# giech/usrp_nfc

Measured on AMD Instinct MI355X. Metric: IQ Msamples/s -> decoded bits (2 Msps stream), higher is better.
Workload: dtype f32 envelope / f64 window sums / u8 symbols; 1 GPU; configs[1]: Miller-only decode, synthetic IQ @2 Msps; input_kind=fc32 IQ, 8 B/sample (envelope computed in the kernel), samples_per_gpu=100000000, parallelism=time-chunk x1, edges_per_gpu=6627699, symbols_reader=3971547, symbols_tag=0, packets=101186, boundary_redos=0, exchange=none, stepping=sync, in_flight=1

## Files before the change

### usrp_nfc_amd/csrc/decode.hip.h

```cpp
#pragma once
#include <hip/hip_runtime.h>
#include <stdint.h>

#include "../../include/nfc_amd.h"
#include "scan.hip.h"

namespace nfc {

struct DecTables {
    const uint4 *mil_map;
    const uint2 *man_map;
    const uint16_t *mil_step;
    const uint16_t *man_step;
    int32_t nd;
    int32_t reader, tag;
    const uint2 *qmil_map;
    const uint16_t *qmil_step;
    uint32_t q_rep[2];
    uint32_t canon[4];
    int32_t q_ok;
};
__device__ __forceinline__ uint32_t byte_of(const uint32_t *w, uint32_t i) { return (w[i >> 2] >> (8u * (i & 3u))) & 0xFFu; }

struct DecCarry {
    int32_t mil_state, man_state;
    int32_t pkt_started[2];
    uint32_t pending[2];
};

constexpr int DEC_ITEMS = 16;
#ifndef NFC_DEC_GROUPS
#define NFC_DEC_GROUPS 2
#endif
constexpr int DEC_GROUPS = NFC_DEC_GROUPS;
constexpr int DEC_PER_THREAD = DEC_ITEMS * DEC_GROUPS;
// ... 337 lines not shown
        v <<= (lo & 31u);
        if (v) atomicOr(dst + w0 + j, v);
    }
}

struct QMaps {
    uint32_t mil[2];
    uint32_t man[2];
};
struct ComposeQ {
    using T = QMaps;
    static __host__ __device__ __forceinline__ T identity() { return T{{0x03020100u, 0x07060504u}, {0x03020100u, 0x07060504u}}; }
    static __device__ __forceinline__ T op(const T &a, const T &b) {
        return T{{__builtin_amdgcn_perm(b.mil[1], b.mil[0], a.mil[0]), __builtin_amdgcn_perm(b.mil[1], b.mil[0], a.mil[1])},
                 {__builtin_amdgcn_perm(b.man[1], b.man[0], a.man[0]), __builtin_amdgcn_perm(b.man[1], b.man[0], a.man[1])}};
    }
    static __device__ __forceinline__ uint32_t step(const T &m, uint32_t st) {
        const uint32_t a = __builtin_amdgcn_perm(m.mil[1], m.mil[0], st & 7u) & 15u;
        const uint32_t b = __builtin_amdgcn_perm(m.man[1], m.man[0], (st >> 4) & 7u) & 15u;
        return a | (b << 4);
    }
};
struct DecSpec {
    QMaps map;
    uint32_t s_in;
    uint32_t needs;
    uint32_t pad[2];
};
static_assert(sizeof(DecSpec) == 32, "two 16-byte loads");
__device__ __forceinline__ bool map8_constant(const uint32_t (&m)[2]) { return m[0] == m[1] && m[0] == (m[0] & 0xFFu) * 0x01010101u; }
constexpr int DEC_RUNIN_MAX = 8;
static_assert(DEC_GROUPS >= 1 && DEC_GROUPS <= 2, "NFC_DEC_GROUPS: a thread's packed bits are accumulated in 64 bits (32 slots per group)");
static_assert(DEC_RUNIN_MAX * SCAN_BLOCK <= DEC_TILE, "the longest run-in fits inside the tile before");
template <bool LDS>
__global__ __launch_bounds__(SCAN_BLOCK) void k_dec_spec(const uint16_t *ecode, size_t n, const uint32_t *n_dev, DecTables T, uint32_t state0, int runin_per_thread,
                                                        uint8_t *outw, FrameAgg *frame_aggs, DecSpec *spec, ZeroJob Z, TileStage S) {
    zero_words(Z);
    if (n_dev) n = min(n, (size_t)*n_dev);
    if ((size_t)blockIdx.x * DEC_TILE >= n) return;
    TP_DECL();
    __shared__ uint2 s_milmap[LDS ? DEC_LDS_ROWS + 1 : 1];
    __shared__ uint2 s_manmap[LDS ? DEC_LDS_ROWS + 1 : 1];
    __shared__ __attribute__((aligned(16))) uint16_t s_mil[LDS ? DEC_LDS_ROWS * 8 : 8];
    __shared__ __attribute__((aligned(16))) uint16_t s_man[LDS ? DEC_LDS_ROWS * 8 : 8];
    __shared__ QMaps lds[SCAN_WAVES];
    __shared__ FramePk lds2[SCAN_WAVES];
    __shared__ uint32_t s_needs;
    __shared__ uint32_t s_bits[2][FW_WORDS];
    __shared__ uint32_t s_drop[2];
    for (int i = threadIdx.x; i < 2 * FW_WORDS; i += SCAN_BLOCK) (&s_bits[0][0])[i] = 0u;
    if (threadIdx.x < 2) s_drop[threadIdx.x] = 0xFFFFFFFFu;
    const uint32_t ident = 4u * (uint32_t)T.nd;
    if (LDS) {
        const int rows = 4 * T.nd;
        for (int i = threadIdx.x; i <= rows; i += SCAN_BLOCK) {
            if (T.reader) s_milmap[i] = T.qmil_map[i];
            if (T.tag) s_manmap[i] = T.man_map[i];
        }
        for (int i = threadIdx.x; i < rows; i += SCAN_BLOCK) {
            if (T.reader) ((uint4 *)s_mil)[i] = ((const uint4 *)T.qmil_step)[i];
            if (T.tag) ((uint4 *)s_man)[i] = ((const uint4 *)T.man_step)[i];
        }
    }
    if (threadIdx.x == 0) s_needs = 0u;
    const size_t tid = (size_t)blockIdx.x * SCAN_BLOCK + threadIdx.x;
    const size_t base = tid * DEC_PER_THREAD;
    uint32_t c[DEC_GROUPS][8];
#pragma unroll
    for (int g = 0; g < DEC_GROUPS; g++) load_codes(ecode, base + DEC_ITEMS * g, n, c[g]);
    uint32_t rc[DEC_RUNIN_MAX / 2];
    const bool have_runin = blockIdx.x > 0;
    {
        const size_t r0 = (size_t)blockIdx.x * DEC_TILE - (size_t)runin_per_thread * SCAN_BLOCK + (size_t)threadIdx.x * runin_per_thread;
#pragma unroll
        for (int k = 0; k < DEC_RUNIN_MAX / 2; k++) rc[k] = (have_runin && 2 * k < runin_per_thread) ? *(const uint32_t *)(ecode + r0 + 2 * k) : 0u;
    }
    __syncthreads();
    TP_MARK();
    auto mil_row = [&](uint32_t code) __attribute__((always_inline)) -> uint2 {
        const uint32_t idx = (code >> 14) == 2u ? (code & 0x3FFFu) : ident;
        return LDS ? s_milmap[idx] : T.qmil_map[idx];
    };
    auto man_row = [&](uint32_t code) __attribute__((always_inline)) -> uint2 {
        const uint32_t idx = (code >> 14) == 1u ? (code & 0x3FFFu) : ident;
        return LDS ? s_manmap[idx] : T.man_map[idx];
    };
    auto then = [](const uint2 &a, const uint2 &b) __attribute__((always_inline)) -> uint2 {
        return make_uint2(__builtin_amdgcn_perm(b.y, b.x, a.x), __builtin_amdgcn_perm(b.y, b.x, a.y));
    };
    auto routes_of = [](uint32_t pair) __attribute__((always_inline)) -> uint32_t {
        const uint32_t r0 = (pair >> 14) & 3u, r1 = pair >> 30;
        return ((r0 == 2u || r1 == 2u) ? 1u : 0u) | ((r0 == 1u || r1 == 1u) ? 2u : 0u);
    };
    auto compose4 = [&](uint2 &am, uint2 &an, uint32_t w0, uint32_t w1) __attribute__((always_inline)) {
        const uint32_t c0 = w0 & 0xFFFFu, c1 = w0 >> 16, c2 = w1 & 0xFFFFu, c3 = w1 >> 16;
        if (T.reader) am = then(am, then(then(mil_row(c0), mil_row(c1)), then(mil_row(c2), mil_row(c3))));
        if (T.tag) an = then(an, then(then(man_row(c0), man_row(c1)), then(man_row(c2), man_row(c3))));
    };
    const QMaps idm = ComposeQ::identity();
    QMaps runin = idm;
    if (have_runin) {
        uint2 am = make_uint2(idm.mil[0], idm.mil[1]), an = make_uint2(idm.man[0], idm.man[1]);
#pragma unroll
        for (int k = 0; k < DEC_RUNIN_MAX / 2; k += 2)
            if (2 * k < runin_per_thread) compose4(am, an, rc[k], rc[k + 1]);
        const QMaps ra{{am.x, am.y}, {an.x, an.y}};
        (void)block_exclusive<ComposeQ>(ra, lds, runin);
    }
    uint32_t seen = 0u;
    uint2 am = make_uint2(idm.mil[0], idm.mil[1]), an = make_uint2(idm.man[0], idm.man[1]);
#ifndef NFC_DEC_CHAIN
#define NFC_DEC_CHAIN 8
#endif
    constexpr int CHAIN = NFC_DEC_CHAIN;
    static_assert(CHAIN == 16 || CHAIN == 8 || CHAIN == 4, "NFC_DEC_CHAIN");
    constexpr int NCH = DEC_PER_THREAD / CHAIN;
    uint2 pm[NCH], pn[NCH];
#pragma unroll
    for (int g = 0; g < DEC_GROUPS; g++) {
#pragma unroll
        for (int k = 0; k < 8; k += 2) {
            if (k % (CHAIN / 2) == 0) {
                pm[(16 * g + 2 * k) / CHAIN] = am;
                pn[(16 * g + 2 * k) / CHAIN] = an;
            }
            compose4(am, an, c[g][k], c[g][k + 1]);
            seen |= routes_of(c[g][k]) | routes_of(c[g][k + 1]);
        }
    }
    if (!T.reader) seen &= ~1u;
    if (!T.tag) seen &= ~2u;
    const QMaps agg{{am.x, am.y}, {an.x, an.y}};
    TP_MARK();
    QMaps total;
    const QMaps excl = block_exclusive<ComposeQ>(agg, lds, total);
    const QMaps upto = ComposeQ::op(runin, excl);
    const uint32_t dep = ((seen & 1u) && !map8_constant(upto.mil) ? 1u : 0u) | ((seen & 2u) && !map8_constant(upto.man) ? 2u : 0u);
    if (blockIdx.x > 0 && dep) atomicOr(&s_needs, dep);
    uint32_t st[NCH];
#pragma unroll
    for (int j = 0; j < NCH; j++) st[j] = ComposeQ::step(ComposeQ::op(upto, QMaps{{pm[j].x, pm[j].y}, {pn[j].x, pn[j].y}}), state0);
    TP_MARK();
    const uint16_t *mil = LDS ? s_mil : T.qmil_step;
    const uint16_t *man = LDS ? s_man : T.man_step;
    uint32_t ow[DEC_GROUPS][4];
#pragma unroll
    for (int g = 0; g < DEC_GROUPS; g++) ow[g][0] = ow[g][1] = ow[g][2] = ow[g][3] = 0u;
#pragma unroll
    for (int e = 0; e < CHAIN; e++) {
#pragma unroll
        for (int j = 0; j < NCH; j++) {
            const int g = (j * CHAIN) / DEC_ITEMS, k = (j * CHAIN) % DEC_ITEMS + e;
            const uint32_t code = (c[g][k >> 1] >> (16 * (k & 1))) & 0xFFFFu;
            const uint32_t li = code & 0x3FFFu, route = code >> 14;
            uint32_t w = 0;
            if (route == 2u && T.reader) {
                const uint32_t en = mil[li * 8u + (st[j] & 7u)];
                w = en >> 8;
                st[j] = (st[j] & ~15u) | (en & 15u);
            } else if (route == 1u && T.tag) {
                const uint32_t en = man[li * 8u + ((st[j] >> 4) & 7u)];
                const uint32_t m = en >> 8;
                w = (m & 3u) ? ((m & 0xFCu) | 3u) : 0u;
                st[j] = (st[j] & 15u) | ((en & 15u) << 4);
            }
            ow[g][k >> 2] |= w << (8 * (k & 3));
        }
    }
    FramePk mine = FramePkOp::identity();
#pragma unroll
    for (int g = 0; g < DEC_GROUPS; g++) {
        const size_t gb = base + (size_t)DEC_ITEMS * g;
        if (gb < n) *(uint4 *)(outw + gb) = make_uint4(ow[g][0], ow[g][1], ow[g][2], ow[g][3]);
        mine = FramePkOp::op(mine, FramePkOp::pack(frame_agg_of(ow[g])));
    }
    TP_MARK();
    FramePk total_fa;
    const FramePk in_tile = block_exclusive<FramePkOp>(mine, lds2, total_fa);
    {
        FrameAgg before = FramePkOp::unpack(in_tile);
        uint64_t acc[2] = {0ull, 0ull};
        uint32_t cnt[2] = {0u, 0u};
        const uint32_t bo0[2] = {before.nb[0], before.nb[1]};
#pragma unroll
        for (int g = 0; g < DEC_GROUPS; g++) {
            if (ow[g][0] | ow[g][1] | ow[g][2] | ow[g][3]) {
                const SlotMasks m = slot_masks(ow[g]);
                const uint32_t low = symbol_low_bits(ow[g]);
#pragma unroll
                for (int t = 0; t < 2; t++) {
                    if (!m.V[t] || !S.bits[t]) continue;
                    const uint32_t started = pm_apply(before.fl[t], 1u);
                    const uint32_t bef = started_before(m, t, started);
                    const uint32_t appended = m.V[t] & ~m.ST[t] & (bef | ~m.SA[t]);
                    uint32_t cl = m.ST[t] & bef;
                    const uint32_t bo = bo0[t] + cnt[t];
                    const uint32_t nonid = m.ST[t] | m.SA[t];
                    if ((before.fl[t] & 3u) == PM_ID && nonid) {
                        const uint32_t first = nonid & (0u - nonid);
                        if (first & m.SA[t]) s_drop[t] = bo + (uint32_t)__popc(appended & (first - 1u));
                    }
                    acc[t] |= (uint64_t)compress32(low, appended) << cnt[t];
                    cnt[t] += (uint32_t)__popc(appended);
                    if (cl) {
                        const uint32_t co = before.nc[t], closes = cl;
                        while (cl) {
                            const uint32_t lowb = cl & (0u - cl);
                            const int k = (__ffs((int)cl) - 1) >> 1;
                            cl ^= lowb;
                            const uint32_t j = co + (uint32_t)__popc(closes & (lowb - 1u));
                            if (j < ST_CLOSES) {
                                const size_t e = base + (size_t)DEC_ITEMS * g + k;
                                S.close_bit[t][(size_t)blockIdx.x * ST_CLOSES + j] = bo + (uint32_t)__popc(appended & (lowb - 1u));
                                S.close_idx[t][(size_t)blockIdx.x * ST_CLOSES + j] = S.idx64 ? S.idx64[e] : S.g0 + (uint64_t)S.epos[e];
                            } else {
                                atomicOr(&s_needs, 4u);
                            }
                        }
                    }
                }
                if (g + 1 < DEC_GROUPS) before = FrameAggOp::op(before, frame_agg_of(ow[g]));
            }
        }
#pragma unroll
        for (int t = 0; t < 2; t++) {
            if (!cnt[t]) continue;
            const uint32_t w = bo0[t] >> 5, sh = bo0[t] & 31u;
            const uint64_t lo = acc[t] << sh;
            const uint32_t hi = sh ? (uint32_t)(acc[t] >> (64u - sh)) : 0u;
            if (w + 2 < (uint32_t)FW_WORDS) {
                if ((uint32_t)lo) atomicOr(&s_bits[t][w], (uint32_t)lo);
                if ((uint32_t)(lo >> 32)) atomicOr(&s_bits[t][w + 1], (uint32_t)(lo >> 32));
                if (hi) atomicOr(&s_bits[t][w + 2], hi);
            }
        }
    }
    __syncthreads();
    const FrameAgg tile_fa = FramePkOp::unpack(total_fa);
#pragma unroll
    for (int t = 0; t < 2; t++) {
        if (!S.bits[t]) continue;
        const uint32_t nw = min((uint32_t)FW_WORDS, (tile_fa.nb[t] + 31u) / 32u + 1u);
        for (uint32_t j = threadIdx.x; j < nw; j += SCAN_BLOCK) S.bits[t][(size_t)blockIdx.x * FW_WORDS + j] = s_bits[t][j];
    }
    if (threadIdx.x == 0) {
        frame_aggs[blockIdx.x] = tile_fa;
        S.own[blockIdx.x] = tile_fa;
        if (S.bits[0]) S.drop_bit[0][blockIdx.x] = s_drop[0];
        if (S.bits[1]) S.drop_bit[1][blockIdx.x] = s_drop[1];
        const uint32_t s_in = ComposeQ::step(runin, state0);
        ((uint4 *)(spec + blockIdx.x))[0] = make_uint4(total.mil[0], total.mil[1], total.man[0], total.man[1]);
        ((uint4 *)(spec + blockIdx.x))[1] = make_uint4(s_in, s_needs, 0u, 0u);
    }
    TP_DONE(1);
}

struct DecVerify {
    const DecSpec *spec;
    uint32_t state0;
    uint32_t q_rep[2];
    DecCarry *carry;
    uint32_t *verdict;
};
constexpr int DV_ITEMS = 4;
__device__ __forceinline__ void dec_verify(const DecVerify &V, size_t ntiles, QMaps *lds) {
    QMaps before = ComposeQ::identity();
    int bad = 0;
    for (size_t b0 = 0; b0 < ntiles; b0 += (size_t)SCAN_BLOCK * DV_ITEMS) {
        const size_t i0 = b0 + (size_t)threadIdx.x * DV_ITEMS;
        QMaps mp[DV_ITEMS];
        uint32_t s_in[DV_ITEMS], needs[DV_ITEMS];
#pragma unroll
        for (int k = 0; k < DV_ITEMS; k++) {
            if (i0 + k < ntiles) {
                const uint4 a = ((const uint4 *)(V.spec + i0 + k))[0], b = ((const uint4 *)(V.spec + i0 + k))[1];
                mp[k] = QMaps{{a.x, a.y}, {a.z, a.w}};
                s_in[k] = b.x;
                needs[k] = b.y;
            } else {
                mp[k] = ComposeQ::identity();
                s_in[k] = 0u;
                needs[k] = 0u;
            }
        }
        QMaps agg = mp[0];
// ... 396 lines not shown
```

### usrp_nfc_amd/csrc/host_context.h

```cpp
#pragma once


namespace {

std::string g_create_error;

__global__ __launch_bounds__(256) void k_certify_and_write(CertLaunch C, EdgeArgs E, size_t nwords, const EdgeAgg *partials, const EdgeAgg *supers,
                                                          uint32_t *epos, uint16_t *ecode, uint32_t cap, bool own_prefix, uint32_t *total_out,
                                                          Last2 *last2_total, EdgeCarry *carry_out) {
    const uint32_t tiles = gridDim.x - C.blocks;
    if (blockIdx.x == 0) {
        certify_block(C.A, C.cert, nullptr, C.ring_next, C.carry, C.sum, C.blocks - 1, C.blocks);
        return;
    }
    if (blockIdx.x > tiles) {
        certify_block(C.A, C.cert, nullptr, C.ring_next, C.carry, C.sum, blockIdx.x - tiles - 1, C.blocks);
        return;
    }
    write_edges_tile(E, nwords, partials, supers, epos, ecode, cap, own_prefix, total_out, last2_total, carry_out, tiles - blockIdx.x, tiles);
}

inline uint64_t &devbuf_allocs() {
    static thread_local uint64_t n = 0;
    return n;
// ... 40 lines not shown
    TOT_EDGES = 8,
    TOT_DECMAP = 16,
    TOT_SPEC = 40,
    TOT_PKT0 = 72,
    TOT_PKT1 = 80,
    TOT_LAST2 = 88,
    TOT_NSYM = 96,
    TOT_CERT = 104,
    TOT_FRAME = 128,
    TOT_BYTES = 160
};

static_assert(sizeof(CertSummary) <= TOT_FRAME - TOT_CERT, "the verdict summary fits its slot of the totals");
struct DevState {
    Carry carry;
    EdgeCarry ecarry;
    DecCarry dcarry;
    uint8_t totals[TOT_BYTES];
    uint32_t seq[4];
};

constexpr size_t AHEAD_LDS_MAX = 96 * 1024;
constexpr int NRING = 4;
constexpr int NSUB = 3;

struct nfc_ctx {
    nfc_params P;
    int L, mx, C, Lpad, wpb, twords;
    double factor;
    double hi_plus, lo_a, lo_b, hi_a, hi_b;
    int bands_ok, fast_ok, nfold, rows_per_step, C_min, wave_slots, lds_per_slot;
    uint32_t ring_carried = 0;
    bool dec_spec = true, dec_spec_now = false;
    int dec_runin = 2, spec_off_left = 0, spec_fail_streak = 0;
    bool bits_packed = false, sym_lazy = false, sym_own = false;
    FrameOut sym_P;
    uint32_t sym_n = 0, sym_tiles = 0;
    uint32_t decode_respeculated = 0;
    int lean = 1, lean_k = 0, lean_rounds = 0, lean_slots = 0;
    int n_cus = 1;
    double rowbal_f[5][3] = {{1, 1, 1}, {1, 1, 1}, {1.02, 1, 1}, {1.045, 1.004, 1}, {1.036, 1.015, 0.990}};
    bool rowbal_set = false;
    bool wg_rowbal = true, rowbal_now = false;
    int wg = 1, wg_ok = 0, wg_nr = 4, wg_slots = 0, wg_slots_ahead = 0, wg_now = 0, wg_rounds = 0;
    int fine_left = 0, fine_adapt = 1, fine_mult = 4;
    size_t wg_lds = 0, wg_lds_base = 0, wg_lds_bulk_max = 0;
    bool wg_bulk = true, wg_bulk_now = false;
    int wg_lone_max = 4, wg_lone_div = 64;
    int wg_rerun_lone = 1;
    int wg_ex_ok = 0, wg_ex_max = 0;
    size_t wg_ex_lds = 0;
    bool wg_ex_launch = false;
    bool wg_flags = false;
    float lean_gfac = 1.3f, lean_gmin = 9.765625e-4f;
    int gring = 0;
    int gring_ok = 0, gring_force = 0, wave_slots_g = 0;
    DevBuf d_gring;
    uint32_t own_prefix_max = OWN_PREFIX_MAX_TILES;
    int use_small = 1;
    double expect_ms = 0.3;
    bool spin_wait = true;
    uint64_t selmask;
    float eps;
    float i16_scale;
    size_t in_bytes_per_sample;
    hipStream_t st = nullptr;
// ... 398 lines not shown
```

### usrp_nfc_amd/csrc/host_stages.h

```cpp
#pragma once

namespace {

int run_edges(nfc_ctx *c, uint32_t n, uint32_t skip, uint64_t g0) {
    uint8_t *tot = dT(c);
    const size_t nwords = ((size_t)n + 63) / 64;
    EdgeArgs E;
    E.neg = c->d_neg.as<uint64_t>();
    E.pos = c->d_pos.as<uint64_t>();
    E.n = n;
    E.skip = skip;
    E.mx = c->mx;
    E.dur_in = c->h_ecarry.dur;
    E.last_bit_in = c->h_ecarry.last_bit;
    E.state_in = c->h_ecarry.state;
    E.nd = c->mx + 1;
    E.g0 = g0;
    E.mx_magic = c->mx > 1 ? (uint32_t)(0x100000000ull / (uint64_t)c->mx) : 0xFFFFFFFFu;
    E.per_mask = 0;
    for (int b = 0; b < 64; b += c->mx) E.per_mask |= 1ull << b;
    E.sw = (uint32_t)(EW_WORDS * EW_SUPER);
    E.tps = (uint32_t)EW_SUPER;
    const size_t tiles = edge_num_tiles(nwords);
    const size_t supers = edge_num_supers(nwords);
// ... 54 lines not shown
        P.pending[t] = c->d_pending[t][c->pend_cur].as<uint8_t>();
        P.pend[t] = pend;
    }
    return NFC_OK;
}

void launch_pkt_finish(nfc_ctx *c, const FrameOut &P, const bool (&enabled)[2], PktCnt *pk_total, FrameAgg *frame_total) {
    const int pn = 1 - c->pend_cur;
    PktFinish F;
    memset(&F, 0, sizeof F);
    F.packed = 1;
    for (int t = 0; t < 2; t++) {
        F.enabled[t] = enabled[t] ? 1 : 0;
        F.bits[t] = P.bits[t];
        F.pending_next[t] = c->d_pending[t][pn].as<uint8_t>();
        F.close_end[t] = P.close_end[t];
        F.started_in[t] = (int32_t)P.started_in[t];
        F.pending_cap[t] = (uint32_t)std::min<size_t>(c->d_pending[t][pn].cap, 0xFFFFFFFFu);
        F.cap_bits[t] = P.cap_bits[t];
        F.cap_close[t] = P.cap_close[t];
    }
    F.totals = pk_total;
    F.frame_total = frame_total;
    F.carry = dD(c);
    static_assert(sizeof(DevState) % 4 == 0, "whole words");
    F.mirror_src = (const uint32_t *)c->d_state.p;
    F.mirror_dst = (uint32_t *)c->hs_dev;
    F.mirror_words = (uint32_t)(sizeof(DevState) / 4);
    F.stamp_word = (uint32_t)(offsetof(DevState, seq) / 4 + 1);
    F.stamp = c->stamp_b;
    NFC_LAUNCH(k_pkt_finish, dim3(1), dim3(256), 0, c->st, F);
}

int run_decode(nfc_ctx *c, bool force_classic = false) {
    uint8_t *tot = dT(c);
    const uint32_t ce = c->cap_edges;
    const uint32_t *ne_dev = (const uint32_t *)(tot + TOT_EDGES);
    const size_t tiles = dec_num_tiles(ce);
    const size_t ce_al = c->edges_from_host ? ce : std::max(ce, c->alloc_edges);
    const size_t tiles_al = dec_num_tiles(ce_al);
    HIPCHK(c, c->d_states.ensure(ce_al + 16));
    HIPCHK(c, c->d_partials.ensure((tiles_al + 1) * sizeof(DecMaps)));
    HIPCHK(c, c->d_partials2.ensure((tiles_al + 1) * sizeof(FrameAgg)));
    HIPCHK(c, c->d_aggs.ensure((tiles_al * SCAN_BLOCK + 1) * sizeof(DecMaps)));
    HIPCHK(c, c->d_faggs.ensure((tiles_al * SCAN_BLOCK + 1) * sizeof(FramePk)));
    const bool enabled[2] = {c->T.tag != 0, c->T.reader != 0};
    FrameOut P;
    const int rf = frame_out(c, P, enabled);
    if (rf) return rf;

    const uint16_t *ecode = c->d_ecode.as<uint16_t>();
    uint8_t *outw = c->d_states.as<uint8_t>();
    const uint32_t dec_state_in = (uint32_t)c->h_dcarry.mil_state | ((uint32_t)c->h_dcarry.man_state << 4);
    const bool lds_tables = 4 * c->T.nd <= DEC_LDS_ROWS;
    DecMaps *dparts = c->d_partials.as<DecMaps>(), *daggs = c->d_aggs.as<DecMaps>();
    FrameAgg *fparts = c->d_partials2.as<FrameAgg>();
    FrameAgg *frame_total = (FrameAgg *)(tot + TOT_FRAME);
    PktCnt *pk_total = (PktCnt *)(tot + TOT_PKT0);
    const bool own = tiles <= c->own_prefix_max;
    DecMaps *map_total = (DecMaps *)(tot + TOT_DECMAP);
    const uint32_t mil_class_in = (c->h_dcarry.mil_state >= 0 && c->h_dcarry.mil_state < 16) ? c->mil_q_of[c->h_dcarry.mil_state] : 0xFFu;
    const bool spec = c->dec_spec && c->spec_off_left == 0 && !force_classic && c->T.q_ok && mil_class_in != 0xFFu;
    c->dec_spec_now = spec;
    DecCarryEpilogue epi{spec ? (DecMaps *)nullptr : map_total, dec_state_in, dD(c), (uint32_t *)(tot + TOT_NSYM), pk_total,
                         {P.pend[0], P.pend[1]}, {P.started_in[0], P.started_in[1]}, {c->T.canon[0], c->T.canon[1], c->T.canon[2], c->T.canon[3]}};
    const uint32_t spec_state_in = mil_class_in | ((uint32_t)c->h_dcarry.man_state << 4);
    DecVerify V{nullptr, spec_state_in, {c->T.q_rep[0], c->T.q_rep[1]}, dD(c), (uint32_t *)(tot + TOT_SPEC)};
    ZeroJob Z;
    for (int t = 0; t < 2; t++) {
        Z.p[t] = (uint32_t *)P.bits[t];
        Z.n[t] = P.bits[t] ? (P.cap_bits[t] + 31u) / 32u + 1u : 0u;
        if (!tiles && Z.n[t]) HIPCHK(c, hipMemsetAsync(Z.p[t], 0, (size_t)Z.n[t] * 4, c->st));
    }
    TileStage S;
    memset(&S, 0, sizeof S);
    if (spec) {
        HIPCHK(c, c->d_spec.ensure((tiles_al + 1) * sizeof(DecSpec)));
        V.spec = c->d_spec.as<DecSpec>();
        HIPCHK(c, c->d_stage_own.ensure((tiles_al + 1) * sizeof(FrameAgg)));
        S.own = c->d_stage_own.as<FrameAgg>();
        S.epos = P.epos;
        S.g0 = P.g0;
        S.idx64 = P.idx64;
        for (int t = 0; t < 2; t++) {
            if (!P.bits[t]) continue;
            HIPCHK(c, c->d_stage_bits[t].ensure((tiles_al + 1) * (size_t)FW_WORDS * 4));
            HIPCHK(c, c->d_stage_cb[t].ensure((tiles_al + 1) * (size_t)ST_CLOSES * 4));
            HIPCHK(c, c->d_stage_ci[t].ensure((tiles_al + 1) * (size_t)ST_CLOSES * 8));
            HIPCHK(c, c->d_stage_q[t].ensure((tiles_al + 1) * 4));
            S.bits[t] = c->d_stage_bits[t].as<uint32_t>();
            S.close_bit[t] = c->d_stage_cb[t].as<uint32_t>();
            S.close_idx[t] = c->d_stage_ci[t].as<uint64_t>();
            S.drop_bit[t] = c->d_stage_q[t].as<uint32_t>();
        }
        if (tiles) {
            if (lds_tables)
                NFC_LAUNCH(k_dec_spec<true>, dim3((unsigned)tiles), dim3(SCAN_BLOCK), 0, c->st, ecode, (size_t)ce, ne_dev, c->T, spec_state_in, c->dec_runin, outw,
                           fparts, c->d_spec.as<DecSpec>(), Z, S);
            else
                NFC_LAUNCH(k_dec_spec<false>, dim3((unsigned)tiles), dim3(SCAN_BLOCK), 0, c->st, ecode, (size_t)ce, ne_dev, c->T, spec_state_in, c->dec_runin, outw,
                           fparts, c->d_spec.as<DecSpec>(), Z, S);
        }
    } else {
        if (tiles) {
            if (lds_tables)
                NFC_LAUNCH(k_dec_reduce<true>, dim3((unsigned)tiles), dim3(SCAN_BLOCK), 0, c->st, ecode, (size_t)ce, ne_dev, c->T, dparts, daggs, Z);
            else
                NFC_LAUNCH(k_dec_reduce<false>, dim3((unsigned)tiles), dim3(SCAN_BLOCK), 0, c->st, ecode, (size_t)ce, ne_dev, c->T, dparts, daggs, Z);
        }
        if (!own) scan_partials<ComposeDec>(c->st, tiles, ne_dev, DEC_TILE, dparts, ComposeDec::identity_host(), map_total);
        if (tiles) {
            if (lds_tables)
                NFC_LAUNCH(k_dec_apply<true>, dim3((unsigned)tiles), dim3(SCAN_BLOCK), 0, c->st, ecode, (size_t)ce, ne_dev, c->T, dparts, daggs,
                                   dec_state_in, outw, fparts, c->d_faggs.as<FramePk>(), own, map_total);
            else
                NFC_LAUNCH(k_dec_apply<false>, dim3((unsigned)tiles), dim3(SCAN_BLOCK), 0, c->st, ecode, (size_t)ce, ne_dev, c->T, dparts, daggs,
                                   dec_state_in, outw, fparts, c->d_faggs.as<FramePk>(), own, map_total);
        }
    }
    if (!own) scan_partials<FrameAggOp>(c->st, tiles, ne_dev, DEC_TILE, fparts, FrameAggOp::identity(), frame_total, epi);
    if (spec)
        NFC_LAUNCH(k_concat, dim3((unsigned)(std::max<size_t>(tiles, 1) + 1)), dim3(SCAN_BLOCK), 0, c->st, (size_t)ce, ne_dev, fparts, S, P, own, frame_total, epi, V);
    else
        NFC_LAUNCH(k_frame_write, dim3((unsigned)std::max<size_t>(tiles, 1)), dim3(SCAN_BLOCK), 0, c->st, outw, (size_t)ce, ne_dev, fparts,
                           c->d_faggs.as<FramePk>(), P, own, frame_total, epi, V);
    c->bits_packed = true;
    c->bits_clean[0] = c->bits_clean[1] = 0;
    c->sym_from_tail = false;
    c->sym_lazy = true;
    c->sym_P = P;
    c->sym_n = ce;
    c->sym_tiles = (uint32_t)tiles;
    c->sym_own = own;
    launch_pkt_finish(c, P, enabled, pk_total, frame_total);
// ... 486 lines not shown
```

### usrp_nfc_amd/csrc/host_submit.h

```cpp
#pragma once

namespace {

bool submit_fast_ok(const nfc_ctx *c, uint32_t n) {
    return c->h_carry.stable && !(c->P.flags & (NFC_FLAG_NO_EDGES | NFC_FLAG_FORCE_SEQUENTIAL)) && c->L >= STEP && c->timing < 2 &&
           !(c->use_small && n <= SM_MAX_SAMPLES) && n > 0 && c->ahead_lds_per_cu <= AHEAD_LDS_MAX && !c->dbg_any && !c->dbg_clk && !c->dbg_no_submit_ahead;
}

int enqueue_threshold_ahead(nfc_ctx *c, nfc_ctx::Submitted &b) {
    if (b.planes < 0) {
        if (!c->alt_free) return fail(c, NFC_ERR_INTERNAL, "no free set of planes");
        b.planes = __builtin_ctz(c->alt_free);
        c->alt_free &= ~(1u << b.planes);
    }
    ThrArgs A;
    ThrPlan P;
    const EdgeCarry unused{0, 0, 0, 0};
    struct AllocNote {
        nfc_ctx::Submitted &b;
        uint64_t a0;
        ~AllocNote() { b.allocs += (uint32_t)(devbuf_allocs() - a0); }
    } alloc_note{b, devbuf_allocs()};
    const nfc_stats keep_stats = c->stats;
    const int rc_prep = thr_prepare(c, b.d_in, b.n, b.n, 0u, 0u, b.g0, unused, b.ring_in, c->d_neg_alt[b.planes], c->d_pos_alt[b.planes], true, A, P);
// ... 44 lines not shown

int enqueue_stages_behind(nfc_ctx *c, nfc_ctx::Submitted &b) {
    struct AllocNote {
        nfc_ctx::Submitted &b;
        uint64_t a0;
        ~AllocNote() { b.allocs += (uint32_t)(devbuf_allocs() - a0); }
    } alloc_note{b, devbuf_allocs()};
    HIPCHK(c, hipStreamWaitEvent(c->st, c->ev_a[b.slot], 0));
    if (b.planes >= 0) take_planes(c, b);
    c->have_outputs = false;
    c->pk_ready[0] = c->pk_ready[1] = false;
    c->n_edges = 0;
    for (int t = 0; t < 2; t++) c->n_sym[t] = c->n_close[t] = c->n_bits[t] = 0;
    memset(&c->stats, 0, sizeof c->stats);
    c->n_kev = 0;
    c->last_n = b.n;
    c->last_g0 = b.g0;
    c->last_skip = 0;
    c->stats.bytes_in = (uint64_t)b.n * c->in_bytes_per_sample;
    c->stats.n_chunks = b.nch;
    c->stats.chunk_samples = b.chunk;
    c->stats.threshold_passes = 1;
    c->stats.ran_ahead = 1;
    c->stamp_b = b.seq;
    c->cert_pending = false;
    size_capacities(c, b.n);
    int rc;
    if (c->tail_on) {
        const bool fused = tail_can_decode(c);
        rc = run_tail(c, b.n, 0u, b.g0);
        if (!rc && !fused) rc = run_decode(c, true);
    } else {
        rc = run_edges(c, b.n, 0u, b.g0);
        if (!rc) rc = run_decode(c);
    }
    if (rc) return rc;
    b.spec = c->dec_spec_now;
    b.tail = c->tail_now;
    HIPCHK(c, hipEventRecord(c->ev_b[b.slot], c->st));
    b.b_enqueued = true;
    return NFC_OK;
}

int restart_submitted(nfc_ctx *c) {
    uint64_t g0 = c->nseen;
    int ring = c->ring_cur;
    bool fast = c->low_valid && !c->state_dirty;
    for (int i = 0; i < c->sub_count; i++) {
        nfc_ctx::Submitted &nb = c->sub[i];
        nb.g0 = g0;
        nb.ring_in = ring;
        nb.b_enqueued = false;
        nb.allocs = 0;
        nb.fast = fast && submit_fast_ok(c, nb.n);
        if (nb.fast) {
            nb.seq = c->batch_seq + 1;
            if (int rc = enqueue_threshold_ahead(c, nb)) return rc;
        }
        if (!nb.fast && nb.planes >= 0) {
            c->alt_free |= 1u << nb.planes;
            nb.planes = -1;
        }
        fast = nb.fast;
        g0 += nb.n;
        ring = (ring + 1) % NRING;
    }
    return NFC_OK;
// ... 221 lines not shown
```

### usrp_nfc_amd/csrc/nfc_amd.hip

```cpp
#include <hip/hip_runtime.h>
#include <hip/hip_ext.h>

#include <algorithm>
#include <atomic>
#include <chrono>
#include <cmath>
#include <cstdarg>
#include <cstdio>
#include <cstdlib>
#include <cstring>
#include <string>
#include <thread>
#include <functional>
#include <vector>

#include "../../include/nfc_amd.h"
#include "launch_check.h"
#include "decode.hip.h"
#include "decoder_tables.h"
#include "edges.hip.h"
#include "protocol.h"
#include "scan.hip.h"
#include "small.hip.h"
#include "threshold.hip.h"
// ... 109 lines not shown
#else
#define NFC_ENV(name) ((const char *)nullptr)
#endif
    c->use_small = NFC_ENV("NFC_NO_SMALL") ? 0 : 1;
#ifdef NFC_TEST_HOOKS
    if (const char *e = getenv("NFC_TAIL")) c->tail_on = atoi(e) != 0;
    c->dbg_bad_launch = getenv("NFC_DEBUG_BAD_LAUNCH") != nullptr;
    c->dbg_redo_submitted = getenv("NFC_DEBUG_REDO_SUBMITTED") != nullptr;
    c->dbg_any = getenv("NFC_DEBUG") != nullptr;
    c->dbg_trace = getenv("NFC_TRACE") != nullptr;
    devbuf_trace() = getenv("NFC_TRACE_ALLOC") != nullptr;
    if (const char *e = getenv("NFC_DEBUG_CLK")) {
        c->dbg_clk = true;
        c->dbg_clk_path = e;
    }
#endif
    c->dbg_no_submit_ahead = NFC_ENV("NFC_NO_SUBMIT_AHEAD") != nullptr;
    if (const char *e = NFC_ENV("NFC_WG")) c->wg = atoi(e) != 0;
    if (const char *e = NFC_ENV("NFC_WG_ROUNDS")) c->wg_rounds = std::max(1, atoi(e));
    if (const char *e = NFC_ENV("NFC_WG_BULK")) c->wg_bulk = atoi(e) != 0;
    if (const char *e = NFC_ENV("NFC_WG_RERUN")) c->wg_rerun_lone = atoi(e) != 0;
    if (const char *e = NFC_ENV("NFC_WG_LONE")) {
        int a = 4, b = 64;
        if (sscanf(e, "%d,%d", &a, &b) >= 1) c->wg_lone_max = std::max(0, a), c->wg_lone_div = std::max(1, b);
    }
    if (const char *e = NFC_ENV("NFC_LEAN")) c->lean = atoi(e) != 0;
    c->lean_k = 0;
    c->lean_rounds = 0;
    if (const char *e = NFC_ENV("NFC_LEAN_ROUNDS")) c->lean_rounds = std::max(1, atoi(e));
    if (const char *e = NFC_ENV("NFC_LEAN_GFAC")) c->lean_gfac = (float)atof(e);
    if (const char *e = NFC_ENV("NFC_LEAN_GMIN")) c->lean_gmin = (float)atof(e);
    if (const char *e = NFC_ENV("NFC_OWN_PREFIX_MAX")) c->own_prefix_max = (uint32_t)strtoul(e, nullptr, 10);
    if (const char *e = NFC_ENV("NFC_DEC_SPEC")) c->dec_spec = atoi(e) != 0;
    if (const char *e = NFC_ENV("NFC_SPIN_WAIT")) c->spin_wait = atoi(e) != 0;
    if (const char *e = NFC_ENV("NFC_WG_ROWBAL")) {
        double f[3];
        f[1] = f[2] = 1.0;
        if (sscanf(e, "%lf,%lf,%lf", &f[0], &f[1], &f[2]) >= 2 && f[0] > 0.5 && f[0] < 1.5 && f[1] > 0.5 && f[1] < 1.5 && f[2] > 0.5 && f[2] < 1.5)
            memcpy(c->rowbal_f[0], f, sizeof f), c->rowbal_set = true;
        else c->wg_rowbal = atoi(e) != 0;
    }
    if (const char *e = NFC_ENV("NFC_DEC_RUNIN")) {
        const int v = atoi(e);
        c->dec_runin = v >= 2048 ? 8 : (v >= 1024 ? 4 : 2);
    }
    {
        c->rows_per_step = 4;
        const int stp = 64 * c->rows_per_step;
        C = (C + stp - 1) / stp * stp;
    }
    c->C = C;
    c->C_min = C;
    c->lds_per_slot = (p->input_kind == NFC_IN_ENV_F32) ? 5 : 4;
    c->wpb = std::max(1, std::min(4, (int)(65536 / ((size_t)c->Lpad * c->lds_per_slot))));
    c->gring_ok = (size_t)c->Lpad * c->lds_per_slot > 12 * 1024 && c->L >= 2 * STEP;
    if (const char *e = NFC_ENV("NFC_RING")) {
        if (strcmp(e, "global") == 0 && c->L >= 2 * STEP) c->gring_ok = c->gring_force = 1;
        else if (strcmp(e, "lds") == 0) c->gring_ok = 0;
    }
    c->hi_plus = p->hi_val + 0.1;
    const double eps = std::ldexp(1.0, -48);
    auto band = [&](double v, double &a, double &b) {
        a = v - std::fabs(v) * eps;
        b = v + std::fabs(v) * eps;
    };
    band(p->lo_val, c->lo_a, c->lo_b);
// ... 1195 lines not shown
```

### usrp_nfc_amd/csrc/scan.hip.h

```cpp
#pragma once
#include <hip/hip_runtime.h>

#include "launch_check.h"
#include <stdint.h>

namespace nfc {

#ifdef NFC_TAIL_PROF
constexpr int TP_WGS = 4096;
#ifndef NFC_HDR_KERNEL_LINKAGE
#define NFC_HDR_KERNEL_LINKAGE
#endif
NFC_HDR_KERNEL_LINKAGE __device__ unsigned long long g_tail_prof[4 * TP_WGS * 8];
#define TP_DECL() unsigned long long tp_t[8]; int tp_n = 0; tp_t[tp_n++] = clock64()
#define TP_MARK() tp_t[tp_n++] = clock64()
#define TP_DONE(slot)                                                                                             \
    do {                                                                                                          \
        tp_t[tp_n++] = clock64();                                                                                 \
        if (threadIdx.x == 0 && blockIdx.x < TP_WGS) {                                                            \
            unsigned long long *o_ = g_tail_prof + ((size_t)(slot) * TP_WGS + blockIdx.x) * 8;                    \
            for (int i_ = 0; i_ < 8; i_++) o_[i_] = i_ < tp_n ? tp_t[i_] : 0ull;                                  \
        }                                                                                                         \
    } while (0)
#else
// ... 92 lines not shown
__device__ __forceinline__ typename Op::T wave_shift_up1_with(const Op &op, const typename Op::T &inc) {
    return dpp_move<0x138, 0xF>(op.identity(), inc);
}
template <class Tr>
__device__ __forceinline__ typename Tr::T wave_shift_up1(const typename Tr::T &inc) {
    return wave_shift_up1_with(StaticOp<Tr>{}, inc);
}

template <int WAVES, class Op>
__device__ __forceinline__ typename Op::T block_exclusive_with(const Op &op, typename Op::T v, typename Op::T *lds,
                                                               typename Op::T &block_total) {
    using T = typename Op::T;
    const int lane = threadIdx.x & 63, wave = threadIdx.x >> 6;
    const T inc = wave_inclusive_with(op, v);
    if (lane == 63) lds[wave] = inc;
    __syncthreads();
    T wave_prefix = op.identity();
    T total = op.identity();
#pragma unroll
    for (int w = 0; w < WAVES; w++) {
        T x = lds[w];
        if (w < wave) wave_prefix = op(wave_prefix, x);
        total = op(total, x);
    }
    __syncthreads();
    block_total = total;
    return op(wave_prefix, wave_shift_up1_with(op, inc));
}
template <class Tr, int WAVES = SCAN_WAVES>
__device__ __forceinline__ typename Tr::T block_exclusive(typename Tr::T v, typename Tr::T *lds,
                                                          typename Tr::T &block_total) {
    return block_exclusive_with<WAVES>(StaticOp<Tr>{}, v, lds, block_total);
}
constexpr uint32_t OWN_PREFIX_MAX_TILES = 4096;
template <int BLOCK, class Op>
__device__ __forceinline__ typename Op::T tile_prefix_with(const Op &op, const typename Op::T *aggs, uint32_t b, typename Op::T *lds) {
    using T = typename Op::T;
    const uint32_t per = (b + BLOCK - 1) / BLOCK;
    const uint32_t lo = min(b, (uint32_t)threadIdx.x * per), hi = min(b, lo + per);
    T acc = op.identity();
    constexpr int G = sizeof(T) <= 8 ? 8 : 4;
    for (uint32_t i = lo; i < hi; i += G) {
        T v[G];
#pragma unroll
        for (int k = 0; k < G; k++) v[k] = (i + k < hi) ? aggs[i + k] : op.identity();
#pragma unroll
        for (int k = 0; k < G; k++) acc = op(acc, v[k]);
    }
    T total;
    (void)block_exclusive_with<BLOCK / 64>(op, acc, lds, total);
    return total;
}
template <class Tr, int BLOCK = 256>
__device__ __forceinline__ typename Tr::T tile_prefix(const typename Tr::T *aggs, uint32_t b, typename Tr::T *lds) {
    return tile_prefix_with<BLOCK>(StaticOp<Tr>{}, aggs, b, lds);
}

constexpr int PART_ITEMS = 8;
struct NoEpilogue {
    template <class T>
    __device__ __forceinline__ void operator()(const T &) const {}
};
template <class Op, int BLOCK, class Epi>
__global__ __launch_bounds__(BLOCK) void k_scan_partials(size_t nparts, const uint32_t *n_dev, uint32_t tile,
                                                        typename Op::T *partials, typename Op::T seed,
                                                        typename Op::T *total_out, Epi epi, Op op) {
// ... 57 lines not shown
```

Measured before the change: 431,300 Msamples/s.

## Add optional wide-block decode kernel with wave0 block scan and dynamic LDS tables

Templates the speculative decode kernel on block size so a tile can be processed by twice as many threads, each holding one group of codes instead of two, with a new wave0-driven block scan for larger blocks. The lookup tables move to dynamically sized shared memory so LDS use matches the real table size. It also adds cheaper route detection, vectorized clearing, and 32-bit accumulators when there is one group. The wide path is off by default (DEC_WIDE_DEFAULT=false) unless NFC_DEC_WIDE is set, so by default only the LDS sizing and micro-tweaks take effect, and those may change occupancy.

```diff
diff --git a/usrp_nfc_amd/csrc/decode.hip.h b/usrp_nfc_amd/csrc/decode.hip.h
--- a/usrp_nfc_amd/csrc/decode.hip.h
+++ b/usrp_nfc_amd/csrc/decode.hip.h
@@ -1,6 +1,8 @@
 #pragma once
 #include <hip/hip_runtime.h>
 #include <stdint.h>
+
+#include <type_traits>
 
 #include "../../include/nfc_amd.h"
 #include "scan.hip.h"
@@ -404,48 +406,72 @@
 constexpr int DEC_RUNIN_MAX = 8;
 static_assert(DEC_GROUPS >= 1 && DEC_GROUPS <= 2, "NFC_DEC_GROUPS: a thread's packed bits are accumulated in 64 bits (32 slots per group)");
 static_assert(DEC_RUNIN_MAX * SCAN_BLOCK <= DEC_TILE, "the longest run-in fits inside the tile before");
-template <bool LDS>
-__global__ __launch_bounds__(SCAN_BLOCK) void k_dec_spec(const uint16_t *ecode, size_t n, const uint32_t *n_dev, DecTables T, uint32_t state0, int runin_per_thread,
-                                                        uint8_t *outw, FrameAgg *frame_aggs, DecSpec *spec, ZeroJob Z, TileStage S) {
+constexpr int DEC_WIDE_BLOCK = DEC_GROUPS == 2 ? 2 * SCAN_BLOCK : SCAN_BLOCK;
+constexpr int dec_min_waves(int block) { return block > SCAN_BLOCK ? 8 : 4; }
+inline size_t dec_table_bytes(const DecTables &T) {
+    const size_t rows = 4 * (size_t)T.nd, ndec = (T.reader ? 1u : 0u) + (T.tag ? 1u : 0u);
+    return ndec * (rows * 16 + (rows + 1) * 8);
+}
+template <bool LDS, int BLOCK>
+__global__ __launch_bounds__(BLOCK, dec_min_waves(BLOCK)) void k_dec_spec(const uint16_t *ecode, size_t n, const uint32_t *n_dev, DecTables T, uint32_t state0, int runin_per_thread,
+                                                                         uint8_t *outw, FrameAgg *frame_aggs, DecSpec *spec, ZeroJob Z, TileStage S) {
+    constexpr int WAVES = BLOCK / 64;
+    constexpr int GROUPS = DEC_TILE / (BLOCK * DEC_ITEMS);
+    constexpr int PER_THREAD = DEC_ITEMS * GROUPS;
+    constexpr int RUNIN_WORDS = DEC_RUNIN_MAX * SCAN_BLOCK / BLOCK / 2;
+    static_assert(GROUPS >= 1 && GROUPS * BLOCK * DEC_ITEMS == DEC_TILE && RUNIN_WORDS >= 2 && RUNIN_WORDS % 2 == 0, "the tile in whole groups, the run-in in whole pairs of words");
     zero_words(Z);
-    if (n_dev) n = min(n, (size_t)*n_dev);
+    if (n_dev) n = min(n, (size_t)(uint32_t)__builtin_amdgcn_readfirstlane((int)*n_dev));
     if ((size_t)blockIdx.x * DEC_TILE >= n) return;
     TP_DECL();
-    __shared__ uint2 s_milmap[LDS ? DEC_LDS_ROWS + 1 : 1];
-    __shared__ uint2 s_manmap[LDS ? DEC_LDS_ROWS + 1 : 1];
-    __shared__ __attribute__((aligned(16))) uint16_t s_mil[LDS ? DEC_LDS_ROWS * 8 : 8];
-    __shared__ __attribute__((aligned(16))) uint16_t s_man[LDS ? DEC_LDS_ROWS * 8 : 8];
-    __shared__ QMaps lds[SCAN_WAVES];
-    __shared__ FramePk lds2[SCAN_WAVES];
-    __shared__ uint32_t s_needs;
-    __shared__ uint32_t s_bits[2][FW_WORDS];
+    extern __shared__ __attribute__((aligned(16))) unsigned char s_dectab[];
+    __shared__ QMaps lds[WAVES + 1];
+    __shared__ FramePk lds2[WAVES + 1];
+    auto scan_q = [&](const QMaps &v, QMaps &tot) __attribute__((always_inline)) -> QMaps {
+        if constexpr (WAVES > SCAN_WAVES) return block_exclusive_by_wave0<ComposeQ, WAVES>(v, lds, tot);
+        else return block_exclusive<ComposeQ, WAVES>(v, lds, tot);
+    };
+    auto scan_f = [&](const FramePk &v, FramePk &tot) __attribute__((always_inline)) -> FramePk {
+        if constexpr (WAVES > SCAN_WAVES) return block_exclusive_by_wave0<FramePkOp, WAVES>(v, lds2, tot);
+        else return block_exclusive<FramePkOp, WAVES>(v, lds2, tot);
+    };
+    __shared__ uint32_t s_needs, s_spec[5];
+    __shared__ __attribute__((aligned(16))) uint32_t s_bits[2][FW_WORDS];
     __shared__ uint32_t s_drop[2];
-    for (int i = threadIdx.x; i < 2 * FW_WORDS; i += SCAN_BLOCK) (&s_bits[0][0])[i] = 0u;
+    static_assert(2 * FW_WORDS % 4 == 0, "cleared four words at a time");
+    for (int i = threadIdx.x; i < 2 * FW_WORDS / 4; i += BLOCK) ((uint4 *)&s_bits[0][0])[i] = make_uint4(0u, 0u, 0u, 0u);
     if (threadIdx.x < 2) s_drop[threadIdx.x] = 0xFFFFFFFFu;
     const uint32_t ident = 4u * (uint32_t)T.nd;
+    const int rows = 4 * T.nd;
+    uint16_t *const s_mil = (uint16_t *)s_dectab;
+    uint16_t *const s_man = s_mil + (T.reader ? rows * 8 : 0);
+    uint2 *const s_milmap = (uint2 *)(s_man + (T.tag ? rows * 8 : 0));
+    uint2 *const s_manmap = s_milmap + (T.reader ? rows + 1 : 0);
     if (LDS) {
-        const int rows = 4 * T.nd;
-        for (int i = threadIdx.x; i <= rows; i += SCAN_BLOCK) {
+        for (int i = threadIdx.x; i <= rows; i += BLOCK) {
             if (T.reader) s_milmap[i] = T.qmil_map[i];
             if (T.tag) s_manmap[i] = T.man_map[i];
         }
-        for (int i = threadIdx.x; i < rows; i += SCAN_BLOCK) {
+        for (int i = threadIdx.x; i < rows; i += BLOCK) {
             if (T.reader) ((uint4 *)s_mil)[i] = ((const uint4 *)T.qmil_step)[i];
             if (T.tag) ((uint4 *)s_man)[i] = ((const uint4 *)T.man_step)[i];
         }
     }
     if (threadIdx.x == 0) s_needs = 0u;
-    const size_t tid = (size_t)blockIdx.x * SCAN_BLOCK + threadIdx.x;
-    const size_t base = tid * DEC_PER_THREAD;
-    uint32_t c[DEC_GROUPS][8];
-#pragma unroll
-    for (int g = 0; g < DEC_GROUPS; g++) load_codes(ecode, base + DEC_ITEMS * g, n, c[g]);
-    uint32_t rc[DEC_RUNIN_MAX / 2];
+    const size_t tid = (size_t)blockIdx.x * BLOCK + threadIdx.x;
+    const size_t base = tid * PER_THREAD;
+    uint32_t c[GROUPS][8];
+#pragma unroll
+    for (int g = 0; g < GROUPS; g++) load_codes(ecode, base + DEC_ITEMS * g, n, c[g]);
+    uint32_t rc[RUNIN_WORDS];
     const bool have_runin = blockIdx.x > 0;
+    const int runin_edges = runin_per_thread * SCAN_BLOCK;
+    const int rpt = max(2, runin_edges / BLOCK);
     {
-        const size_t r0 = (size_t)blockIdx.x * DEC_TILE - (size_t)runin_per_thread * SCAN_BLOCK + (size_t)threadIdx.x * runin_per_thread;
-#pragma unroll
-        for (int k = 0; k < DEC_RUNIN_MAX / 2; k++) rc[k] = (have_runin && 2 * k < runin_per_thread) ? *(const uint32_t *)(ecode + r0 + 2 * k) : 0u;
+        const bool takes = have_runin && (int)threadIdx.x * rpt < runin_edges;
+        const size_t r0 = (size_t)blockIdx.x * DEC_TILE - (size_t)runin_edges + (size_t)threadIdx.x * rpt;
+#pragma unroll
+        for (int k = 0; k < RUNIN_WORDS; k++) rc[k] = (takes && 2 * k < rpt) ? *(const uint32_t *)(ecode + r0 + 2 * k) : 0u;
     }
     __syncthreads();
     TP_MARK();
@@ -460,9 +486,9 @@
     auto then = [](const uint2 &a, const uint2 &b) __attribute__((always_inline)) -> uint2 {
         return make_uint2(__builtin_amdgcn_perm(b.y, b.x, a.x), __builtin_amdgcn_perm(b.y, b.x, a.y));
     };
-    auto routes_of = [](uint32_t pair) __attribute__((always_inline)) -> uint32_t {
-        const uint32_t r0 = (pair >> 14) & 3u, r1 = pair >> 30;
-        return ((r0 == 2u || r1 == 2u) ? 1u : 0u) | ((r0 == 1u || r1 == 1u) ? 2u : 0u);
+    auto routes_of = [](uint32_t pair) __attribute__((always_inline)) -> uint2 {
+        const uint32_t r = pair >> 14;
+        return make_uint2((r >> 1) & ~r & 0x00010001u, r & ~(r >> 1) & 0x00010001u);
     };
     auto compose4 = [&](uint2 &am, uint2 &an, uint32_t w0, uint32_t w1) __attribute__((always_inline)) {
         const uint32_t c0 = w0 & 0xFFFFu, c1 = w0 >> 16, c2 = w1 & 0xFFFFu, c3 = w1 >> 16;
@@ -474,22 +500,22 @@
     if (have_runin) {
         uint2 am = make_uint2(idm.mil[0], idm.mil[1]), an = make_uint2(idm.man[0], idm.man[1]);
 #pragma unroll
-        for (int k = 0; k < DEC_RUNIN_MAX / 2; k += 2)
-            if (2 * k < runin_per_thread) compose4(am, an, rc[k], rc[k + 1]);
+        for (int k = 0; k < RUNIN_WORDS; k += 2)
+            if (2 * k < rpt) compose4(am, an, rc[k], rc[k + 1]);
         const QMaps ra{{am.x, am.y}, {an.x, an.y}};
-        (void)block_exclusive<ComposeQ>(ra, lds, runin);
-    }
-    uint32_t seen = 0u;
+        (void)scan_q(ra, runin);
+    }
+    uint32_t any_mil = 0u, any_man = 0u;
     uint2 am = make_uint2(idm.mil[0], idm.mil[1]), an = make_uint2(idm.man[0], idm.man[1]);
 #ifndef NFC_DEC_CHAIN
 #define NFC_DEC_CHAIN 8
 #endif
     constexpr int CHAIN = NFC_DEC_CHAIN;
     static_assert(CHAIN == 16 || CHAIN == 8 || CHAIN == 4, "NFC_DEC_CHAIN");
-    constexpr int NCH = DEC_PER_THREAD / CHAIN;
+    constexpr int NCH = PER_THREAD / CHAIN;
     uint2 pm[NCH], pn[NCH];
 #pragma unroll
-    for (int g = 0; g < DEC_GROUPS; g++) {
+    for (int g = 0; g < GROUPS; g++) {
 #pragma unroll
         for (int k = 0; k < 8; k += 2) {
             if (k % (CHAIN / 2) == 0) {
@@ -497,27 +523,37 @@
                 pn[(16 * g + 2 * k) / CHAIN] = an;
             }
             compose4(am, an, c[g][k], c[g][k + 1]);
-            seen |= routes_of(c[g][k]) | routes_of(c[g][k + 1]);
-        }
-    }
+            const uint2 ra = routes_of(c[g][k]), rb = routes_of(c[g][k + 1]);
+            any_mil |= ra.x | rb.x;
+            any_man |= ra.y | rb.y;
+        }
+    }
+    uint32_t seen = ((any_mil | (any_mil >> 16)) & 1u) | (((any_man | (any_man >> 16)) & 1u) << 1);
     if (!T.reader) seen &= ~1u;
     if (!T.tag) seen &= ~2u;
     const QMaps agg{{am.x, am.y}, {an.x, an.y}};
     TP_MARK();
     QMaps total;
-    const QMaps excl = block_exclusive<ComposeQ>(agg, lds, total);
+    const QMaps excl = scan_q(agg, total);
     const QMaps upto = ComposeQ::op(runin, excl);
     const uint32_t dep = ((seen & 1u) && !map8_constant(upto.mil) ? 1u : 0u) | ((seen & 2u) && !map8_constant(upto.man) ? 2u : 0u);
     if (blockIdx.x > 0 && dep) atomicOr(&s_needs, dep);
+    if (threadIdx.x == 0) {
+        s_spec[0] = total.mil[0];
+        s_spec[1] = total.mil[1];
+        s_spec[2] = total.man[0];
+        s_spec[3] = total.man[1];
+        s_spec[4] = ComposeQ::step(runin, state0);
+    }
     uint32_t st[NCH];
 #pragma unroll
     for (int j = 0; j < NCH; j++) st[j] = ComposeQ::step(ComposeQ::op(upto, QMaps{{pm[j].x, pm[j].y}, {pn[j].x, pn[j].y}}), state0);
     TP_MARK();
     const uint16_t *mil = LDS ? s_mil : T.qmil_step;
     const uint16_t *man = LDS ? s_man : T.man_step;
-    uint32_t ow[DEC_GROUPS][4];
-#pragma unroll
-    for (int g = 0; g < DEC_GROUPS; g++) ow[g][0] = ow[g][1] = ow[g][2] = ow[g][3] = 0u;
+    uint32_t ow[GROUPS][4];
+#pragma unroll
+    for (int g = 0; g < GROUPS; g++) ow[g][0] = ow[g][1] = ow[g][2] = ow[g][3] = 0u;
 #pragma unroll
     for (int e = 0; e < CHAIN; e++) {
 #pragma unroll
@@ -541,21 +577,26 @@
     }
     FramePk mine = FramePkOp::identity();
 #pragma unroll
-    for (int g = 0; g < DEC_GROUPS; g++) {
+    for (int g = 0; g < GROUPS; g++) {
         const size_t gb = base + (size_t)DEC_ITEMS * g;
         if (gb < n) *(uint4 *)(outw + gb) = make_uint4(ow[g][0], ow[g][1], ow[g][2], ow[g][3]);
         mine = FramePkOp::op(mine, FramePkOp::pack(frame_agg_of(ow[g])));
     }
     TP_MARK();
     FramePk total_fa;
-    const FramePk in_tile = block_exclusive<FramePkOp>(mine, lds2, total_fa);
+    const FramePk in_tile = scan_f(mine, total_fa);
+    if (BLOCK > SCAN_BLOCK) {
+#pragma unroll
+        for (int g = 0; g < GROUPS; g++) asm volatile("" : "+v"(ow[g][0]), "+v"(ow[g][1]), "+v"(ow[g][2]), "+v"(ow[g][3]));
+    }
     {
         FrameAgg before = FramePkOp::unpack(in_tile);
-        uint64_t acc[2] = {0ull, 0ull};
+        using Acc = typename std::conditional<GROUPS == 1, uint32_t, uint64_t>::type;
+        Acc acc[2] = {0u, 0u};
         uint32_t cnt[2] = {0u, 0u};
         const uint32_t bo0[2] = {before.nb[0], before.nb[1]};
 #pragma unroll
-        for (int g = 0; g < DEC_GROUPS; g++) {
+        for (int g = 0; g < GROUPS; g++) {
             if (ow[g][0] | ow[g][1] | ow[g][2] | ow[g][3]) {
                 const SlotMasks m = slot_masks(ow[g]);
                 const uint32_t low = symbol_low_bits(ow[g]);
@@ -572,7 +613,7 @@
                         const uint32_t first = nonid & (0u - nonid);
                         if (first & m.SA[t]) s_drop[t] = bo + (uint32_t)__popc(appended & (first - 1u));
                     }
-                    acc[t] |= (uint64_t)compress32(low, appended) << cnt[t];
+                    acc[t] |= (Acc)compress32(low, appended) << cnt[t];
                     cnt[t] += (uint32_t)__popc(appended);
                     if (cl) {
                         const uint32_t co = before.nc[t], closes = cl;
@@ -591,15 +632,15 @@
                         }
                     }
                 }
-                if (g + 1 < DEC_GROUPS) before = FrameAggOp::op(before, frame_agg_of(ow[g]));
+                if (g + 1 < GROUPS) before = FrameAggOp::op(before, frame_agg_of(ow[g]));
             }
         }
 #pragma unroll
         for (int t = 0; t < 2; t++) {
             if (!cnt[t]) continue;
             const uint32_t w = bo0[t] >> 5, sh = bo0[t] & 31u;
-            const uint64_t lo = acc[t] << sh;
-            const uint32_t hi = sh ? (uint32_t)(acc[t] >> (64u - sh)) : 0u;
+            const uint64_t lo = (uint64_t)acc[t] << sh;
+            const uint32_t hi = (GROUPS > 1 && sh) ? (uint32_t)((uint64_t)acc[t] >> (64u - sh)) : 0u;
             if (w + 2 < (uint32_t)FW_WORDS) {
                 if ((uint32_t)lo) atomicOr(&s_bits[t][w], (uint32_t)lo);
                 if ((uint32_t)(lo >> 32)) atomicOr(&s_bits[t][w + 1], (uint32_t)(lo >> 32));
@@ -613,16 +654,15 @@
     for (int t = 0; t < 2; t++) {
         if (!S.bits[t]) continue;
         const uint32_t nw = min((uint32_t)FW_WORDS, (tile_fa.nb[t] + 31u) / 32u + 1u);
-        for (uint32_t j = threadIdx.x; j < nw; j += SCAN_BLOCK) S.bits[t][(size_t)blockIdx.x * FW_WORDS + j] = s_bits[t][j];
+        for (uint32_t j = threadIdx.x; j < nw; j += BLOCK) S.bits[t][(size_t)blockIdx.x * FW_WORDS + j] = s_bits[t][j];
     }
     if (threadIdx.x == 0) {
         frame_aggs[blockIdx.x] = tile_fa;
         S.own[blockIdx.x] = tile_fa;
         if (S.bits[0]) S.drop_bit[0][blockIdx.x] = s_drop[0];
         if (S.bits[1]) S.drop_bit[1][blockIdx.x] = s_drop[1];
-        const uint32_t s_in = ComposeQ::step(runin, state0);
-        ((uint4 *)(spec + blockIdx.x))[0] = make_uint4(total.mil[0], total.mil[1], total.man[0], total.man[1]);
-        ((uint4 *)(spec + blockIdx.x))[1] = make_uint4(s_in, s_needs, 0u, 0u);
+        ((uint4 *)(spec + blockIdx.x))[0] = make_uint4(s_spec[0], s_spec[1], s_spec[2], s_spec[3]);
+        ((uint4 *)(spec + blockIdx.x))[1] = make_uint4(s_spec[4], s_needs, 0u, 0u);
     }
     TP_DONE(1);
 }
diff --git a/usrp_nfc_amd/csrc/host_context.h b/usrp_nfc_amd/csrc/host_context.h
--- a/usrp_nfc_amd/csrc/host_context.h
+++ b/usrp_nfc_amd/csrc/host_context.h
@@ -96,6 +96,7 @@
     int bands_ok, fast_ok, nfold, rows_per_step, C_min, wave_slots, lds_per_slot;
     uint32_t ring_carried = 0;
     bool dec_spec = true, dec_spec_now = false;
+    int dec_wide = -1;
     int dec_runin = 2, spec_off_left = 0, spec_fail_streak = 0;
     bool bits_packed = false, sym_lazy = false, sym_own = false;
     FrameOut sym_P;
diff --git a/usrp_nfc_amd/csrc/host_stages.h b/usrp_nfc_amd/csrc/host_stages.h
--- a/usrp_nfc_amd/csrc/host_stages.h
+++ b/usrp_nfc_amd/csrc/host_stages.h
@@ -110,7 +110,10 @@
     NFC_LAUNCH(k_pkt_finish, dim3(1), dim3(256), 0, c->st, F);
 }
 
-int run_decode(nfc_ctx *c, bool force_classic = false) {
+constexpr bool DEC_WIDE_DEFAULT = false;
+constexpr size_t DEC_WIDE_MIN_TILES = 4;
+constexpr bool DEC_WIDE_AHEAD = true;
+int run_decode(nfc_ctx *c, bool force_classic = false, bool submitted = false) {
     uint8_t *tot = dT(c);
     const uint32_t ce = c->cap_edges;
     const uint32_t *ne_dev = (const uint32_t *)(tot + TOT_EDGES);
@@ -172,12 +175,20 @@
             S.drop_bit[t] = c->d_stage_q[t].as<uint32_t>();
         }
         if (tiles) {
-            if (lds_tables)
-                NFC_LAUNCH(k_dec_spec<true>, dim3((unsigned)tiles), dim3(SCAN_BLOCK), 0, c->st, ecode, (size_t)ce, ne_dev, c->T, spec_state_in, c->dec_runin, outw,
-                           fparts, c->d_spec.as<DecSpec>(), Z, S);
-            else
-                NFC_LAUNCH(k_dec_spec<false>, dim3((unsigned)tiles), dim3(SCAN_BLOCK), 0, c->st, ecode, (size_t)ce, ne_dev, c->T, spec_state_in, c->dec_runin, outw,
-                           fparts, c->d_spec.as<DecSpec>(), Z, S);
+            const bool wide = DEC_WIDE_BLOCK != SCAN_BLOCK &&
+                              (c->dec_wide >= 0 ? c->dec_wide != 0 : DEC_WIDE_DEFAULT && tiles > DEC_WIDE_MIN_TILES && (!submitted || DEC_WIDE_AHEAD));
+            const size_t dyn = lds_tables ? dec_table_bytes(c->T) : 0;
+#define NFC_DEC_SPEC_LAUNCH(LDS, BLOCK)                                                                                                             \
+    NFC_LAUNCH((k_dec_spec<LDS, BLOCK>), dim3((unsigned)tiles), dim3(BLOCK), dyn, c->st, ecode, (size_t)ce, ne_dev, c->T, spec_state_in, c->dec_runin, outw, \
+               fparts, c->d_spec.as<DecSpec>(), Z, S)
+            if (wide) {
+                if (lds_tables) NFC_DEC_SPEC_LAUNCH(true, DEC_WIDE_BLOCK);
+                else NFC_DEC_SPEC_LAUNCH(false, DEC_WIDE_BLOCK);
+            } else {
+                if (lds_tables) NFC_DEC_SPEC_LAUNCH(true, SCAN_BLOCK);
+                else NFC_DEC_SPEC_LAUNCH(false, SCAN_BLOCK);
+            }
+#undef NFC_DEC_SPEC_LAUNCH
         }
     } else {
         if (tiles) {
diff --git a/usrp_nfc_amd/csrc/host_submit.h b/usrp_nfc_amd/csrc/host_submit.h
--- a/usrp_nfc_amd/csrc/host_submit.h
+++ b/usrp_nfc_amd/csrc/host_submit.h
@@ -100,7 +100,7 @@
         if (!rc && !fused) rc = run_decode(c, true);
     } else {
         rc = run_edges(c, b.n, 0u, b.g0);
-        if (!rc) rc = run_decode(c);
+        if (!rc) rc = run_decode(c, false, true);
     }
     if (rc) return rc;
     b.spec = c->dec_spec_now;
diff --git a/usrp_nfc_amd/csrc/nfc_amd.hip b/usrp_nfc_amd/csrc/nfc_amd.hip
--- a/usrp_nfc_amd/csrc/nfc_amd.hip
+++ b/usrp_nfc_amd/csrc/nfc_amd.hip
@@ -165,6 +165,7 @@
     if (const char *e = NFC_ENV("NFC_LEAN_GMIN")) c->lean_gmin = (float)atof(e);
     if (const char *e = NFC_ENV("NFC_OWN_PREFIX_MAX")) c->own_prefix_max = (uint32_t)strtoul(e, nullptr, 10);
     if (const char *e = NFC_ENV("NFC_DEC_SPEC")) c->dec_spec = atoi(e) != 0;
+    if (const char *e = NFC_ENV("NFC_DEC_WIDE")) c->dec_wide = atoi(e) != 0 ? 1 : 0;
     if (const char *e = NFC_ENV("NFC_SPIN_WAIT")) c->spin_wait = atoi(e) != 0;
     if (const char *e = NFC_ENV("NFC_WG_ROWBAL")) {
         double f[3];
diff --git a/usrp_nfc_amd/csrc/scan.hip.h b/usrp_nfc_amd/csrc/scan.hip.h
--- a/usrp_nfc_amd/csrc/scan.hip.h
+++ b/usrp_nfc_amd/csrc/scan.hip.h
@@ -148,6 +148,36 @@
                                                           typename Tr::T &block_total) {
     return block_exclusive_with<WAVES>(StaticOp<Tr>{}, v, lds, block_total);
 }
+template <int WAVES, class Op>
+__device__ __forceinline__ typename Op::T block_exclusive_by_wave0_with(const Op &op, typename Op::T v, typename Op::T *lds,
+                                                                        typename Op::T &block_total) {
+    using T = typename Op::T;
+    static_assert(WAVES >= 2 && WAVES <= 16, "the wave totals fill one row of 16 lanes at most");
+    const int lane = threadIdx.x & 63, wave = __builtin_amdgcn_readfirstlane((int)(threadIdx.x >> 6));
+    const T id = op.identity();
+    const T inc = wave_inclusive_with(op, v);
+    if (lane == 63) lds[wave] = inc;
+    __syncthreads();
+    if (wave == 0) {
+        T x = lane < WAVES ? lds[lane] : id;
+        x = op(dpp_move<0x111, 0xF>(id, x), x);
+        if (WAVES > 2) x = op(dpp_move<0x112, 0xF>(id, x), x);
+        if (WAVES > 4) x = op(dpp_move<0x114, 0xF>(id, x), x);
+        if (WAVES > 8) x = op(dpp_move<0x118, 0xF>(id, x), x);
+        const T ex = wave_shift_up1_with(op, x);
+        if (lane < WAVES) lds[lane] = ex;
+        if (lane == WAVES - 1) lds[WAVES] = x;
+    }
+    __syncthreads();
+    const T wave_prefix = lds[wave];
+    block_total = lds[WAVES];
+    __syncthreads();
+    return op(wave_prefix, wave_shift_up1_with(op, inc));
+}
+template <class Tr, int WAVES>
+__device__ __forceinline__ typename Tr::T block_exclusive_by_wave0(typename Tr::T v, typename Tr::T *lds, typename Tr::T &block_total) {
+    return block_exclusive_by_wave0_with<WAVES>(StaticOp<Tr>{}, v, lds, block_total);
+}
 constexpr uint32_t OWN_PREFIX_MAX_TILES = 4096;
 template <int BLOCK, class Op>
 __device__ __forceinline__ typename Op::T tile_prefix_with(const Op &op, const typename Op::T *aggs, uint32_t b, typename Op::T *lds) {
```

Result: no change. 427,900 Msamples/s (-0.8%).
